# TiagoBsCastro/SLICER

Measured on AMD Instinct MI355X. Metric: particles/s deposited (TSC, 4096^2 map), higher is better.
Workload: dtype f32; 1 GPU; 512^3-particle GADGET-2 boxes (8 sub-files), 4 snapshots resident in HBM, 4096^2 TSC, 4 lens planes per pass, uniform; algo=auto, accum=f32, algo_mask=84, streams=1

## Files before the change

slicer_amd/csrc/binned_pass.cpp:

```cpp
#include "slicer_host.hpp"

#include <algorithm>
#include <cmath>
#include <cstring>

using namespace slicer;

namespace {

size_t acc_elem_size(int kind) { return (kind == kF64 || kind == kFixed64) ? 8 : 4; }

int zero_flush(slicer_handle h)
{
    ZeroList &Z = h->zero_list;
    if (Z.n == 1) {
        HIPCHK(h, hipMemsetAsync(Z.p[0], 0, Z.words[0] * 4, h->stream));
    } else if (Z.n > 1) {
        HIPCHK(h, launch_zero_many(Z, h->stream));
    }
    Z.n = 0;
    Z.quad0[0] = 0;
    return SLICER_OK;
}

// ... 83 lines not shown
                if (rc)
                    return rc;
                rc = zero_async(h, h->planes[p].acc[type].p, b);
                if (rc)
                    return rc;
            }
        }
        h->type_seen[type] = true;
    }
    return SLICER_OK;
}


int scatter_workgroups(slicer_handle h)
{
    return h->num_cus * std::max(1, h->opt.k3_per_cu);
}

int ensure_bin_workspace(slicer_handle h, bool has_mass, int group, int slot, uint64_t n, const BinGeom &G,
                         BinWorkspace &W)
{
    auto &Q = h->pg[group];
    const uint64_t nb = (n + G.batch - 1) / G.batch;
    const uint64_t region = (uint64_t)G.n_units * nb * G.region;
    const uint64_t nrec = n * (uint64_t)(G.region / G.batch);
    int rc;
    if ((rc = ensure(h, h->w_cxy, region * 8)) || (rc = ensure(h, h->w_cbin, region * 2)) ||
        (rc = ensure(h, h->w_hist, nb * (uint64_t)G.nbins * 4)) ||
        (rc = ensure(h, h->w_hist16, nb * (uint64_t)(G.nbins + 2) * 2)) ||
        (rc = ensure(h, h->w_total, (kMaxBins + kMaxBins / 32 + 1) * 4)) ||
        (rc = ensure(h, h->w_bcount, nb * kMaxUnits * 4)) || (rc = ensure(h, Q.w_sxy[slot], nrec * (has_mass ? 12 : 8))) ||
        (rc = ensure(h, Q.w_base[slot], (kMaxBins + 1) * 4)))
        return rc;
    if (has_mass && (rc = ensure(h, h->w_cm, region * 4)))
        return rc;
    W.cxy = (float2 *)h->w_cxy.p;
    W.cbin = (unsigned short *)h->w_cbin.p;
    W.cm = (float *)h->w_cm.p;
    W.sxy = (float2 *)Q.w_sxy[slot].p;
    W.sm = has_mass ? (float *)Q.w_sxy[slot].p : nullptr;
    W.hist = (unsigned *)h->w_hist.p;
    W.hist16 = (unsigned *)h->w_hist16.p;
    W.total = (unsigned *)h->w_total.p;
    W.base = (unsigned *)Q.w_base[slot].p;
    W.bcount = (unsigned *)h->w_bcount.p;
    return SLICER_OK;
}

bool sort2_geom(const BinGeom &G, int n_planes, BinGeom &G2, int &crow_log2)
{
    G2 = G;
    crow_log2 = 0;
    auto units = [&](int cl) { return n_planes * ((G.nty + (1 << cl) - 1) >> cl); };
    while (units(crow_log2) > 64 && (2 << crow_log2) * G.ntx <= kMaxCoarseTiles)
        crow_log2++;
    G2.rows_per_unit = 1 << crow_log2;
    G2.units_per_plane = (G.nty + G2.rows_per_unit - 1) / G2.rows_per_unit;
    G2.tiles_per_unit = G2.rows_per_unit * G.ntx;
    G2.n_units = n_planes * G2.units_per_plane;
    G2.nbins = G2.n_units * G2.tiles_per_unit;
    return G2.n_units <= kMaxCoarse && G2.tiles_per_unit <= kMaxCoarseTiles && G.region == G.batch && G.batch <= 32768;
// ... 326 lines not shown
```

slicer_amd/csrc/slicer_capi.cpp:

```cpp
#include "slicer_host.hpp"

#include <algorithm>
#include <cmath>
#include <cstdlib>
#include <cstring>
#include <new>

using namespace slicer;

namespace {

int env_int(const char *name, int dflt = 0)
{
    const char *v = getenv(name);
    return v && *v ? atoi(v) : dflt;
}

int copy_map_to_host(slicer_handle h, void *dst, const void *d_src, size_t bytes)
{
    HIPCHK(h, hipMemcpy(dst, d_src, bytes, hipMemcpyDeviceToHost));
    return SLICER_OK;
}

}
// ... 107 lines not shown
}

int slicer_destroy(slicer_handle h)
{
    if (!h)
        return SLICER_OK;
    (void)hipSetDevice(h->device);
    (void)hipStreamSynchronize(h->stream);
    prof_collect(h);
    thin_drop(h);
    pass_stream_return(h);
    for (auto e : h->ev_pool)
        (void)hipEventDestroy(e);
    for (auto &pl : h->planes) {
        release(pl.tot);
        release(pl.acc_shared);
        for (int t = 0; t < 6; t++) {
            release(pl.toti[t]);
            release(pl.acc[t]);
        }
    }
    if (h->d_sweep)
        (void)hipFree(h->d_sweep);
    for (DevBuf *b : {&h->w_cxy, &h->w_cbin, &h->w_cm, &h->w_hist, &h->w_hist16, &h->w_total, &h->w_bcount, &h->w_items,
                      &h->w_tcounts, &h->w_tbase, &h->w_urand, &h->w_randtab, &h->w_randstate, &h->w_randwaves, &h->w_c1, &h->w_sboff, &h->w_sbstart, &h->w_sbn})
        release(*b);
    for (auto &Q : h->pg) {
        release(Q.w_tot);
        for (int i = 0; i < kMaxPending; i++) {
            release(Q.w_sxy[i]);
            release(Q.w_base[i]);
            release(Q.w_ptab[i]);
        }
    }
    for (int i = 0; i < 2; i++) {
        if (h->h_stage[i]) (void)hipHostFree(h->h_stage[i]);
        if (h->d_stage[i]) (void)hipFree(h->d_stage[i]);
        if (h->h_mstage[i]) (void)hipHostFree(h->h_mstage[i]);
        if (h->d_mstage[i]) (void)hipFree(h->d_mstage[i]);
        if (h->stage_free[i]) (void)hipEventDestroy(h->stage_free[i]);
    }
    if (h->d_counts) (void)hipFree(h->d_counts);
    if (h->own) (void)hipStreamDestroy(h->own);
    delete h;
    return SLICER_OK;
}

// ... 484 lines not shown
```

slicer_amd/csrc/slicer_host.hpp:

```cpp
#pragma once
#include <hip/hip_runtime.h>

#include <cstdint>
#include <string>
#include <utility>
#include <vector>

#include "../../include/slicer_amd.h"
#include "slicer_kernels.hpp"

#pragma GCC visibility push(hidden)

struct DevBuf {
    void *p = nullptr;
    size_t cap = 0;
};

struct PlaneBufs {
    DevBuf tot;
    DevBuf toti[6];
    DevBuf acc[6];
    DevBuf acc_shared;
};

// ... 68 lines not shown
    unsigned long long *d_counts = nullptr;
    int *d_neg = nullptr;
    unsigned *d_maxmass = nullptr;
    bool type_seen[6] = {};
    bool shared_seen = false;
    int algo_mask = 0;
    bool neg_remote = false;
    int file_mode[6] = {};
    bool file_partial_flush[6] = {};
    unsigned file_serial = 0;
    float file_mconst[6] = {};
    int fixed_exp[6] = {};
    int fixed_exp_shared = 0;
    bool fixed_exp_set[6] = {};
    bool fixed_shared_set = false;

    float *h_stage[2] = {nullptr, nullptr};
    float *d_stage[2] = {nullptr, nullptr};
    float *h_mstage[2] = {nullptr, nullptr};
    float *d_mstage[2] = {nullptr, nullptr};
    hipEvent_t stage_free[2] = {nullptr, nullptr};
    uint64_t stage_cap = 0;

    DevBuf w_cxy, w_cbin, w_cm, w_hist, w_hist16, w_total, w_bcount, w_items;
    DevBuf w_c1, w_sboff, w_sbstart, w_sbn;
    std::vector<std::pair<double, bool>> box_verdicts;
    std::vector<std::pair<int, bool>> dl_verdicts;
    bool dl_quot_ok = false;
    unsigned *d_sweep = nullptr;
    DevBuf w_tcounts, w_tbase, w_urand;
    std::vector<float> h_urand;
    DevBuf w_randtab, w_randstate, w_randwaves;
    bool rand_tab_ready = false;
    bool rand_on_device = false;
    slicer::ZeroList zero_list{};
    bool zero_collect = false;
    bool rand_private = false;
    uint32_t rand_state[31] = {};
    bool rand_pass = false;
    struct ThinChunk {
        int file, type;
        DevBuf pos, mass;
        uint64_t n;
    };
    struct ThinFile {
        slicer_file_desc file;
        int mode[6];
// ... 96 lines not shown
```

slicer_amd/csrc/slicer_kernels.hpp:

```cpp
#pragma once
#include <hip/hip_runtime.h>
#include <stdint.h>

#include "slicer_device.hpp"

namespace slicer {

enum Mas { kTSC = 0, kNGP = 1 };
enum Acc { kF32 = 0, kF64 = 1, kFixed64 = 2, kCountU32 = 3,
           kF32I = 4, kF64I = 5 };

struct Targets {
    void *acc[kMaxPlanes];
    unsigned long long *nsel[kMaxPlanes];
    int *neg_flag;
    unsigned *max_mass;
};

struct LaunchCfg {
    int mas;
    int acc;
    bool has_mass;
};

hipError_t launch_direct(const LaunchCfg &cfg, const float *d_pos, const float *d_mass, uint64_t n,
                         const PassParams &P, const Targets &T, hipStream_t s);
// ... 53 lines not shown
                                int *neg_flag, hipStream_t s);

struct BinGeom {
    int tw_log2, th_log2;
    int ntx, nty;
    int tiles_per_unit;
    int units_per_plane;
    int rows_per_unit;
    int n_units;
    int nbins;
    int batch;
    int region;
};
constexpr int kMaxUnits = 32;
constexpr int kMaxBins = 32768;

struct BinWorkspace {
    float2 *c1;
    unsigned *sb_off, *sb_n;
    unsigned short *sb_start;
    unsigned *ptab;
    unsigned *item_tot;
    unsigned *tot;
    float2 *cxy;
    unsigned short *cbin;
    float *cm;
    float2 *sxy;
    float *sm;
    unsigned *hist16;
    unsigned *hist;
    unsigned *total;
    unsigned *base;
    unsigned *bcount;
};

struct K1Args {
    const float *pos;
    const float *mass;
    uint64_t n;
    float2 *cxy;
    unsigned short *cbin;
    float *cm;
    unsigned *hist16;
    unsigned *bcount;
    int *neg_flag;
    unsigned long long *nsel;
    float rb, boxf;
    float ws[3], wo[3];
    float c0f[3];
    float rcase;
    int face;
    float zlo[4], zlast;
    int n_planes, vec, ngp;
    int stack;
    float k_ra, eps_ra, k_dec, eps_dec;
    double series_max, lim, inv_fov;
    double nn_d;
    float nn_f;
    int nn;
    int pow2;
    int tw_log2, th_log2, ntx, tiles_per_unit, units_per_plane, rows_per_unit, n_units, nbins, batch;
    int ntx_log2, tpu_log2;
    int sort2, crow_log2;
    float2 *c1;
    unsigned *sb_off;
// ... 61 lines not shown
```

slicer_amd/csrc/slicer_project_bin.hip:

```cpp
#include "slicer_binned_common.hpp"

#pragma clang fp contract(off)

namespace slicer {

namespace {

#ifndef SLICER_K1_BLOCK
#define SLICER_K1_BLOCK 512
#endif
#ifndef SLICER_K1_WAVES_PER_SIMD
#define SLICER_K1_WAVES_PER_SIMD 4
#endif
constexpr int kK1Block = SLICER_K1_BLOCK;
#ifndef SLICER_K1_PER_THREAD
#define SLICER_K1_PER_THREAD 4
#endif
constexpr int kPerThread = SLICER_K1_PER_THREAD;
static_assert(kPerThread == 4 || kPerThread == 2, "load_round handles 2 or 4 particles per lane");
constexpr int kRound = kK1Block * kPerThread;
constexpr int kWaves = kK1Block / 64;
constexpr int kWaveQ = 64 * kPerThread + 64;

struct RawRound {
// ... 159 lines not shown
        A.sb_off[sg] = blockIdx.x * (unsigned)A.batch + off;
    lds_barrier();
    if (tid < nu)
        St.cnt[tid] = 0;
    if (tid == 3 * 64)
        *St.n = 0;
    float2 *out = A.c1 + (size_t)blockIdx.x * (size_t)A.batch + off;
    for (unsigned j = tid; j < n; j += kK1Block)
        out[j] = St.rec[St.perm[j]];
    off += n;
    slot++;
    lds_barrier();
}

enum { kEmitGeneric = 0,
       kEmitLean = 1,
       kEmitSort2 = 2,
       kEmitLeanNgp = 3,
       kEmitLeanMass = 4 };

template <int MODE, bool POW2>
__device__ __forceinline__ void emit_record(const K1Args &A, unsigned *s_hist, unsigned *s_out, unsigned *s_cnt, bool valid,
                                            int plane, float xs, float ys, int gx, int gy, unsigned idx_in_batch,
                                            uint64_t b0, float2 *out_wg, unsigned unit_stride)
{
    constexpr bool LEAN = MODE == kEmitLean || MODE == kEmitLeanNgp || MODE == kEmitLeanMass;
    const bool ngp = MODE == kEmitLeanNgp || (!LEAN && A.ngp != 0);
    const int nn = A.nn;
    bool emit = valid;
    if (ngp) {
        emit = valid && gx >= 0 && gx < nn && gy >= 0 && gy < nn;
        if (valid && !emit)
            atomicAdd(&s_cnt[plane], 1u);
    }
    gx = min(max(gx, 0), nn - 1);
    gy = min(max(gy, 0), nn - 1);
    if (MODE == kEmitSort2 || (MODE == kEmitGeneric && A.sort2)) {
        const Stage St = stage_of(s_hist);
        const unsigned coarse = (unsigned)plane * (unsigned)A.units_per_plane + ((unsigned)(gy >> A.th_log2) >> A.crow_log2);
        const unsigned long long em = __ballot(emit);
        if (em != 0ull) {
            const int lead = (int)__builtin_ctzll(em);
            unsigned base = 0;
            if ((int)lane_id() == lead)
                base = atomicAdd(St.n, (unsigned)__popcll(em));
            base = (unsigned)__builtin_amdgcn_readlane((int)base, lead);
            if (emit) {
                const unsigned idx = base + (unsigned)__popcll(em & ((1ull << lane_id()) - 1ull));
                const unsigned r = atomicAdd(&St.cnt[coarse], 1u);
                St.rec[idx] = make_float2(xs, ys);
                St.bin[idx] = (unsigned char)coarse;
                St.rank[idx] = (unsigned short)r;
            }
        }
        return;
    }
    if (emit) {
        const unsigned ty = (unsigned)(gy >> A.th_log2), tx = (unsigned)(gx >> A.tw_log2);
        unsigned band = 0, trow = ty;
        if (!LEAN && A.units_per_plane > 1) {
            band = ty / (unsigned)A.rows_per_unit;
            trow = ty - band * (unsigned)A.rows_per_unit;
        }
        const unsigned unit = LEAN ? (unsigned)plane : (unsigned)plane * (unsigned)A.units_per_plane + band;
        const bool shifts = LEAN && POW2;
        const unsigned tile_in_unit = shifts ? (trow << A.ntx_log2) | tx : trow * (unsigned)A.ntx + tx;
        const unsigned bin = shifts ? (unit << A.tpu_log2) | tile_in_unit : unit * (unsigned)A.tiles_per_unit + tile_in_unit;
        const unsigned o = atomicAdd(&s_out[unit], 1u);
        const unsigned idx = unit * unit_stride + o;
        out_wg[idx] = make_float2(xs, ys);
        A.cbin[(size_t)blockIdx.x * (size_t)A.batch + idx] = (unsigned short)tile_in_unit;
        if (MODE == kEmitLeanMass || (!LEAN && A.mass != nullptr))
            A.cm[(size_t)blockIdx.x * (size_t)A.batch + idx] = A.mass[b0 + idx_in_batch];
        atomicAdd(&s_hist[bin >> 1], 1u << ((bin & 1u) * 16u));
    }
}

__device__ SLICER_SLOWPATH bool process_exact(const K1Kernarg *Kk, unsigned *s_hist, unsigned *s_out, unsigned *s_cnt,
                                              unsigned idx_in_batch, uint64_t b0, float2 *out_wg, unsigned unit_stride)
{
    const PassParams P = Kk->P;
    const K1Args A = Kk->A;
    const float *r = A.pos + 3 * (b0 + idx_in_batch);
    float x, y, z;
    transform(r[0], r[1], r[2], P, x, y, z);
    const bool neg = (x < 0.0f) | (y < 0.0f) | (z < 0.0f);
    for (int p = 0; p < P.n_planes; p++) {
        if (!(z >= P.zlo[p] && z < P.zhi[p]))
            continue;
        float xs, ys;
        if (project<0>(x, y, z, 0, 0, P, xs, ys)) {
            const int gx = P.pow2 ? grid_index<true>(xs, P) : grid_index<false>(xs, P);
            const int gy = P.pow2 ? grid_index<true>(ys, P) : grid_index<false>(ys, P);
            emit_record<kEmitGeneric, false>(A, s_hist, s_out, s_cnt, true, p, xs, ys, gx, gy, idx_in_batch, b0, out_wg, unit_stride);
        }
    }
    return neg;
}

template <bool POW2, int MODE>
__device__ __forceinline__ void decide_emit(const K1Args &A, unsigned *s_hist, unsigned *s_out, unsigned *s_cnt,
                                            unsigned *s_exc, unsigned *s_nexc, bool have, float ez, double sn, double tn,
                                            double dec, double ra, unsigned tag, uint64_t b0, float2 *out_wg,
                                            unsigned unit_stride)
{
    float xs = 0.f, ys = 0.f;
    const double adec = fabs(dec), ara = fabs(ra);
    const double sx = fma(dec, A.inv_fov, 0.5), sy = fma(ra, A.inv_fov, 0.5);
    const bool dx = round_decided(sx, kMapWindow, xs), dy = round_decided(sy, kMapWindow, ys);
    bool undecided = !(fabs(sn) <= A.series_max && fabs(tn) <= A.series_max && ez > 0.0f) ||
                     fabs(adec - A.lim) <= kAngWindow || fabs(ara - A.lim) <= kAngWindow || !dx || !dy;
    int gx, gy;
    if (POW2) {
        gx = (int)floorf(xs * A.nn_f);
        gy = (int)floorf(ys * A.nn_f);
    } else {
        const double tx = (double)xs * A.nn_d, ty = (double)ys * A.nn_d;
        const double fx = floor(tx), fy = floor(ty);
        undecided = undecided || tx == fx || ty == fy;
        gx = (int)fx;
        gy = (int)fy;
    }
    if (have && undecided)
        s_exc[min(atomicAdd(s_nexc, 1u), kExcCap - 1)] = tag >> 3;
    const bool valid = have && !undecided && adec <= A.lim && ara <= A.lim;
    emit_record<MODE, POW2>(A, s_hist, s_out, s_cnt, valid, (int)(tag & 7u), xs, ys, gx, gy, tag >> 3, b0, out_wg, unit_stride);
}

template <int SERIES, bool POW2, int MODE>
__device__ __forceinline__ void project_emit(const K1Args &A, unsigned *s_hist, unsigned *s_out, unsigned *s_cnt,
                                             unsigned *s_exc, unsigned *s_nexc, bool have, float ex, float ey, float ez,
                                             unsigned tag, uint64_t b0, float2 *out_wg, unsigned unit_stride)
{
    const double X = (double)ex - 0.5, Y = (double)ey - 0.5, Z = (double)ez;
    const double R2 = fma(Y, Y, Z * Z);
    const double sn = X * rsqrt_fast(R2);
    const double tn = Y * rcp_fast(Z);
    double dec, ra;
    atan_small_pair<SERIES>(sn, tn, dec, ra);
    decide_emit<POW2, MODE>(A, s_hist, s_out, s_cnt, s_exc, s_nexc, have, ez, sn, tn, dec, ra, tag, b0, out_wg, unit_stride);
}

template <int SERIES, bool POW2, int MODE>
__device__ __forceinline__ void project_emit2(const K1Args &A, unsigned *s_hist, unsigned *s_out, unsigned *s_cnt,
                                              unsigned *s_exc, unsigned *s_nexc, const bool *have, const float *ex,
                                              const float *ey, const float *ez, const unsigned *tag, uint64_t b0, float2 *out_wg, unsigned unit_stride)
{
    double t[4], ang[4];
#pragma unroll
    for (int j = 0; j < 2; j++) {
        const double X = (double)ex[j] - 0.5, Y = (double)ey[j] - 0.5, Z = (double)ez[j];
        const double R2 = fma(Y, Y, Z * Z);
        t[2 * j] = X * rsqrt_fast(R2);
        t[2 * j + 1] = Y * rcp_fast(Z);
    }
    atan_small_quad<SERIES>(t, ang);
#pragma unroll
    for (int j = 0; j < 2; j++)
        decide_emit<POW2, MODE>(A, s_hist, s_out, s_cnt, s_exc, s_nexc, have[j], ez[j], t[2 * j], t[2 * j + 1], ang[2 * j],
                          ang[2 * j + 1], tag[j], b0, out_wg, unit_stride);
}

template <int FACE, int SERIES, bool STACK, bool POW2, int MODE>
__global__ __launch_bounds__(kK1Block, SLICER_K1_WAVES_PER_SIMD) void k_project_bin_fast(K1Kernarg K)
{
    constexpr bool SORT2 = MODE == kEmitSort2;
    static_assert(!(STACK && SORT2), "the two-level sort runs without the wave stacks");
    const K1Args &A = K.A;
    extern __shared__ __attribute__((aligned(16))) unsigned smem[];
// ... 11 lines not shown
        s_hist[i] = 0;
    if (tid < kMaxPlanes)
        s_cnt[tid] = 0;
    if (tid < kMaxUnits)
        s_out[tid] = 0;
    if (tid == 0) {
        s_neg = 0;
        s_nexc = 0;
    }
    if (SORT2) {
        const Stage St = stage_of(smem);
        if (tid < kMaxCoarse) {
            St.cnt[tid] = 0;
            St.tot[tid] = 0;
        }
        if (tid == 0)
            *St.n = 0;
    }
    __syncthreads();
    unsigned st_off = 0, st_slot = 0;

    const uint64_t b0 = (uint64_t)blockIdx.x * A.batch;
    const uint64_t b1 = dmin<uint64_t>(A.n, b0 + A.batch);
    float2 *const out_wg = A.cxy + (size_t)blockIdx.x * (size_t)A.batch;
    const unsigned unit_stride = gridDim.x * (unsigned)A.batch;
    unsigned top = 0;

    const uint64_t w0 = b0 + (uint64_t)wave * (64 * kPerThread);
    RawRound cur;
    const __amdgpu_buffer_rsrc_t rsrc = batch_rsrc(A.pos, b0, b1);
    uint64_t i0 = w0 + (uint64_t)kPerThread * lane;
    int nvalid = i0 < b1 ? (int)dmin<uint64_t>(kPerThread, b1 - i0) : 0;
    load_round(rsrc, (unsigned)(i0 - b0), cur);

    const uint64_t lim = SORT2 ? b1 + (w0 - b0) : b1;
    for (uint64_t r0 = w0; r0 < lim; r0 += kRound) {
        const uint64_t i1 = i0 + kRound;
        const bool more = r0 + kRound < lim;
        const int nvalid1 = (more && i1 < b1) ? (int)dmin<uint64_t>(kPerThread, b1 - i1) : 0;

        static_assert(kPerThread % 2 == 0, "particles are projected in pairs");
        float px[kPerThread], py[kPerThread], pz[kPerThread];
        bool psel[kPerThread];
        unsigned ptag[kPerThread];
        {
#pragma unroll
            for (int k = 0; k < kPerThread; k++) {
// ... 117 lines not shown
                atomicAdd(&A.item_tot[(size_t)(blockIdx.x / kSort2Blocks) * A.n_units + tid], c);
                atomicAdd(&s_cnt[tid / A.units_per_plane], c);
            }
        }
        __syncthreads();
        if (tid < A.n_planes && s_cnt[tid])
            atomicAdd(A.nsel + 6 * tid, (unsigned long long)s_cnt[tid]);
        return;
    }
    unsigned *row = A.hist16 + (size_t)blockIdx.x * hist_words;
    for (int i = tid; i < hist_words; i += kK1Block)
        row[i] = s_hist[i];
    if (tid < A.n_units)
        A.bcount[(size_t)tid * gridDim.x + blockIdx.x] = s_out[tid];
    if (tid == 0 && s_neg)
        atomicOr(A.neg_flag, 1);
    if (A.ngp && tid < A.n_planes && s_cnt[tid])
        atomicAdd(A.nsel + 6 * tid, (unsigned long long)s_cnt[tid]);
}

template <int MAS, bool POW2, bool HAS_MASS, int SERIES, bool REP>
__global__ __launch_bounds__(kK1Block, SLICER_K1_WAVES_PER_SIMD) void k_project_bin_general(
    const float *__restrict__ pos, const float *__restrict__ mass, uint64_t n, int vec, PassParams P, BinGeom G,
    float2 *__restrict__ cxy, unsigned short *__restrict__ cbin, float *__restrict__ cm, unsigned *__restrict__ hist16,
    unsigned *__restrict__ bcount, Targets T)
{
    extern __shared__ unsigned smem[];
    unsigned *s_hist = smem;
    const int hist_words = (G.nbins + 1) >> 1;
    const int tid = threadIdx.x;
    const unsigned lane = lane_id();
    const int wave = tid >> 6;
    float4 *q4 = reinterpret_cast<float4 *>(smem + ((hist_words + 3) & ~3)) + (size_t)wave * kWaveQ;
    __shared__ unsigned s_out[kMaxUnits], s_cnt[kMaxPlanes];
    __shared__ int s_neg;

    for (int i = tid; i < hist_words; i += kK1Block)
        s_hist[i] = 0;
    if (tid < kMaxPlanes)
        s_cnt[tid] = 0;
    if (tid < kMaxUnits)
        s_out[tid] = 0;
    if (tid == 0)
        s_neg = 0;
    __syncthreads();

    const uint64_t b0 = (uint64_t)blockIdx.x * G.batch;
// ... 29 lines not shown
                    valid = true;
                    int gx = grid_index<POW2>(xs, P);
                    int gy = grid_index<POW2>(ys, P);
                    const int nn = P.nn;
                    if (MAS == kNGP) {
                        emit = gx >= 0 && gx < nn && gy >= 0 && gy < nn;
                    } else {
                        emit = true;
                        gx = gx < 0 ? 0 : (gx >= nn ? nn - 1 : gx);
                        gy = gy < 0 ? 0 : (gy >= nn ? nn - 1 : gy);
                    }
                    cell_to_tile(gx, gy, plane, G, unit, tile_in_unit);
                    bin = unit * (unsigned)G.tiles_per_unit + tile_in_unit;
                    if (HAS_MASS)
                        m = mass[b0 + (tag >> 10)];
                }
            }
            top -= take;
            if (MAS == kNGP && valid && !emit)
                atomicAdd(&s_cnt[plane], 1u);
            if (emit) {
                const unsigned o = atomicAdd(&s_out[unit], 1u);
                const uint64_t dst = ((uint64_t)unit * gridDim.x + blockIdx.x) * (uint64_t)G.region + o;
                cxy[dst] = make_float2(xs, ys);
                cbin[dst] = (unsigned short)tile_in_unit;
                if (HAS_MASS)
                    cm[dst] = m;
                atomicAdd(&s_hist[bin >> 1], 1u << ((bin & 1u) * 16u));
            }
        }
    };

    for (uint64_t r0 = w0; r0 < b1; r0 += kRound) {
        const uint64_t i1 = i0 + kRound;
        const bool more = r0 + kRound < b1;
        const int nvalid1 = (more && i1 < b1) ? (int)dmin<uint64_t>(kPerThread, b1 - i1) : 0;
        load_round(rsrc, (unsigned)(i1 - b0), nxt);

        if (!REP) {
#pragma unroll
            for (int k = 0; k < kPerThread; k++) {
                float x, y, z;
                transform(cur.v[3 * k], cur.v[3 * k + 1], cur.v[3 * k + 2], P, x, y, z);
                const bool live = k < nvalid;
                neg |= live & ((x < 0.0f) | (y < 0.0f) | (z < 0.0f));
                int pl = -1;
                if (P.n_planes <= 4) {
#pragma unroll
                    for (int p = 0; p < 4; p++)
                        if (z >= P.zlo[p] && z < P.zhi[p])
// ... 158 lines not shown
            if (s9) K1F(9, false, kEmitLeanMass); else K1F(15, false, kEmitLeanMass);
        } else if (lean) {
            if (s9) K1F(9, false, kEmitLean); else K1F(15, false, kEmitLean);
        } else {
            if (s9) K1F(9, false, kEmitGeneric); else K1F(15, false, kEmitGeneric);
        }
    }
#undef K1F_
#undef K1F
    return hipGetLastError();
}

template <int MAS, bool POW2, bool HAS_MASS, int SERIES>
static hipError_t launch_k1_general(bool vec, const float *pos, const float *mass, uint64_t n, const PassParams &P,
                                    const BinGeom &G, const BinWorkspace &W, const Targets &T, hipStream_t s)
{
    const int nb = (int)((n + G.batch - 1) / G.batch);
    const size_t lds = project_bin_lds_bytes(G, HAS_MASS);
    hipError_t e;
    if (G.region != G.batch) {
        auto kern = k_project_bin_general<MAS, POW2, HAS_MASS, SERIES, true>;
        if ((e = set_lds(kern, lds)) != hipSuccess)
            return e;
        kern<<<nb, kK1Block, lds, s>>>(pos, mass, n, vec ? 1 : 0, P, G, W.cxy, W.cbin, W.cm, W.hist16, W.bcount, T);
    } else {
        auto kern = k_project_bin_general<MAS, POW2, HAS_MASS, SERIES, false>;
        if ((e = set_lds(kern, lds)) != hipSuccess)
            return e;
        kern<<<nb, kK1Block, lds, s>>>(pos, mass, n, vec ? 1 : 0, P, G, W.cxy, W.cbin, W.cm, W.hist16, W.bcount, T);
    }
    return hipGetLastError();
}

hipError_t launch_project_bin(const LaunchCfg &cfg, bool fast, const float *d_pos, const float *d_mass, uint64_t n,
                              const PassParams &P, const K1Args &A0, const BinGeom &G, const BinWorkspace &W,
                              const Targets &T, hipStream_t s)
{
    const bool vec = (reinterpret_cast<uintptr_t>(d_pos) & 15u) == 0 && (G.batch % 4) == 0;
    const bool pow2 = P.pow2 != 0;
    bool s9 = P.series_max < 0.2;
    if (fast) {
        s9 = A0.series_max < 0.2;
        K1Args A = A0;
        A.pos = d_pos;
        A.mass = cfg.has_mass ? d_mass : nullptr;
        A.n = n;
        A.vec = vec ? 1 : 0;
        A.ngp = cfg.mas == kNGP;
        A.cxy = W.cxy;
        A.cbin = W.cbin;
        A.cm = W.cm;
        A.hist16 = W.hist16;
        A.bcount = W.bcount;
        A.neg_flag = T.neg_flag;
        A.nsel = T.nsel[0];
        A.tw_log2 = G.tw_log2, A.th_log2 = G.th_log2, A.ntx = G.ntx, A.tiles_per_unit = G.tiles_per_unit;
        auto log2_exact = [](int v) {
            int l = 0;
            while ((1 << l) < v)
                l++;
            return (1 << l) == v ? l : -1;
        };
        A.ntx_log2 = log2_exact(G.ntx), A.tpu_log2 = log2_exact(G.tiles_per_unit);
        A.units_per_plane = G.units_per_plane, A.rows_per_unit = G.rows_per_unit, A.n_units = G.n_units;
        A.nbins = G.nbins, A.batch = G.batch;
        A.c1 = W.c1;
        A.sb_off = W.sb_off;
        A.sb_start = W.sb_start;
        A.sb_n = W.sb_n;
        A.item_tot = W.item_tot;
        if (A.sort2)
            A.stack = 0;
        const int nb = (int)((n + G.batch - 1) / G.batch);
        const size_t lds = A.sort2 ? project_bin_sort2_lds_bytes() : project_bin_lds_bytes(G, cfg.has_mass);
// ... 25 lines not shown
```

slicer_amd/csrc/slicer_sort.hip:

```cpp
#include "slicer_binned_common.hpp"

#pragma clang fp contract(off)

namespace slicer {


constexpr int kScanBins = 32;
constexpr int kScanSegs = 1024 / kScanBins;

__global__ __launch_bounds__(1024) void k_scan_blocks(const unsigned short *__restrict__ hist16,
                                                      unsigned *__restrict__ prefix, unsigned *__restrict__ lex,
                                                      unsigned *__restrict__ gsum, int nblocks, int nbins)
{
    __shared__ unsigned s_seg[kScanSegs][kScanBins];
    const int bl = threadIdx.x % kScanBins, seg = threadIdx.x / kScanBins;
    const int bin = blockIdx.x * kScanBins + bl;
    const size_t stride16 = (size_t)((nbins + 1) >> 1) * 2;
    const int per = (nblocks + kScanSegs - 1) / kScanSegs;
    const int lo = seg * per, hi = lo + per < nblocks ? lo + per : nblocks;
    constexpr int kKeep = 16;
    unsigned short keep[kKeep];
    const bool kept = per <= kKeep;
    unsigned sum = 0;
    if (bin < nbins) {
// ... 37 lines not shown
            const unsigned y = (unsigned)__shfl_up((int)x, d, kScanBins);
            if (bl >= d)
                x += y;
        }
        if (bin < nbins)
            lex[bin] = x - tot;
        if (bl == kScanBins - 1)
            gsum[blockIdx.x] = x;
    }
}

#ifndef SLICER_K3_BLOCK
#define SLICER_K3_BLOCK 512
#endif
constexpr int kSortBlock = SLICER_K3_BLOCK;
constexpr int kSortBatch = 8192;
#ifndef SLICER_K3_STAGE
#define SLICER_K3_STAGE 4096
#endif
#ifndef SLICER_K3_WAVES
#define SLICER_K3_WAVES 4
#endif
constexpr int kSortStage = SLICER_K3_STAGE;

__device__ __forceinline__ unsigned block_exclusive_scan(unsigned v, unsigned *s_wave )
{
    unsigned x = v;
#pragma unroll
    for (int d = 1; d < 64; d <<= 1) {
        const unsigned y = (unsigned)__shfl_up((int)x, d);
        if ((int)lane_id() >= d)
            x += y;
    }
    const int w = threadIdx.x >> 6;
    if (lane_id() == 63)
        s_wave[w] = x;
    lds_barrier();
    unsigned off = 0;
    for (int k = 0; k < w; k++)
        off += s_wave[k];
    lds_barrier();
    return off + x - v;
}

template <bool HAS_MASS>
__global__ __launch_bounds__(kSortBlock, SLICER_K3_WAVES) void k_bin_scatter(const float2 *__restrict__ cxy,
                                                            const unsigned short *__restrict__ cbin,
                                                            const float *__restrict__ cm,
                                                            const unsigned *__restrict__ hist16w,
                                                            const unsigned *__restrict__ prefix,
                                                            const unsigned *__restrict__ lex,
                                                            const unsigned *__restrict__ gsum,
                                                            unsigned *__restrict__ base,
                                                            const unsigned *__restrict__ bcount, int nblocks,
                                                            BinGeom G, float2 *__restrict__ sxy,
                                                            float *__restrict__ sm, int count_planes, Targets T)
{
    extern __shared__ unsigned smem_sc[];
    const int tpp = G.tiles_per_unit;
    const int tw = (tpp + 1) >> 1;
    unsigned *cnt = smem_sc;
    unsigned *pos = cnt + tw;
    unsigned *cur = pos + tpp;
    float2 *sorted_xy = reinterpret_cast<float2 *>(cur + tpp + (tw & 1));
    unsigned short *sorted_tile = reinterpret_cast<unsigned short *>(sorted_xy + kSortStage);
    float *sorted_m = reinterpret_cast<float *>(sorted_tile + kSortStage);
    __shared__ unsigned s_wave[kSortBlock / 64];
    __shared__ unsigned s_gp[kMaxBins / kScanBins + 1];

    const int tid = threadIdx.x;
    {
// ... 14 lines not shown
                s_gp[g] = e;
            e += v[j];
        }
        if (tid == kSortBlock - 1)
            s_gp[ngroups] = e;
        lds_barrier();
        if (blockIdx.x == 0) {
            for (int i = tid; i <= G.nbins; i += kSortBlock)
                base[i] = i < G.nbins ? s_gp[i / kScanBins] + lex[i] : s_gp[ngroups];
            if (tid < count_planes) {
                const int bpp = G.units_per_plane * G.tiles_per_unit;
                auto at = [&](int i) { return i < G.nbins ? s_gp[i / kScanBins] + lex[i] : s_gp[ngroups]; };
                const unsigned c = at((tid + 1) * bpp) - at(tid * bpp);
                if (c)
                    atomicAdd(T.nsel[tid], (unsigned long long)c);
            }
        }
    }
    const int per_unit = 8 * ((nblocks + 7) / 8);
    const int per_xcd = per_unit / 8;
    const int per = (tpp + kSortBlock - 1) / kSortBlock;
    auto get16 = [](const unsigned *tab, unsigned t) { return (tab[t >> 1] >> ((t & 1u) * 16u)) & 0xFFFFu; };
    constexpr int R = kSortBatch / kSortBlock;
    float mass_max = 0.0f;
    for (int item = blockIdx.x; item < G.n_units * per_unit; item += gridDim.x) {
        const int plane = item / per_unit;
        const int u = item % per_unit;
        const int lb = (u & 7) * per_xcd + (u >> 3);
        if (lb >= nblocks)
            continue;
        const unsigned count = bcount[(size_t)plane * nblocks + lb];
        if (count == 0)
            continue;
        lds_barrier();
        const unsigned *row = prefix + (size_t)lb * G.nbins + (size_t)plane * tpp;
        const unsigned *lrow = lex + (size_t)plane * tpp;
        const unsigned bin0 = (unsigned)plane * (unsigned)tpp;
        for (int i = tid; i < tpp; i += kSortBlock)
            cur[i] = s_gp[(bin0 + (unsigned)i) / kScanBins] + lrow[i] + row[i];
        const uint64_t r0 = ((uint64_t)plane * nblocks + lb) * (uint64_t)G.region;

        const bool single = count <= (unsigned)kSortBatch && (((unsigned)plane * (unsigned)tpp) & 1u) == 0u;
        for (unsigned s0 = 0; s0 < count; s0 += kSortBatch) {
            const unsigned nsub = count - s0 < (unsigned)kSortBatch ? count - s0 : (unsigned)kSortBatch;
            if (!single) {
                for (int i = tid; i < tw; i += kSortBlock)
                    cnt[i] = 0;
                lds_barrier();
            }
            unsigned tile[R];
            float2 xy[R];
            float m[R];
#pragma unroll
            for (int k = 0; k < R; k++) {
                const unsigned i = (unsigned)k * kSortBlock + tid;
                if (i < nsub) {
                    tile[k] = cbin[r0 + s0 + i];
                    xy[k] = cxy[r0 + s0 + i];
                    if (HAS_MASS)
                        m[k] = cm[r0 + s0 + i];
                    if (!single)
                        atomicAdd(&cnt[tile[k] >> 1], 1u << ((tile[k] & 1u) * 16u));
                }
            }
            if (single) {
                const unsigned *hrow =
                    hist16w + (size_t)lb * (size_t)((G.nbins + 1) >> 1) + (((size_t)plane * tpp) >> 1);
                for (int i = tid; i < tw; i += kSortBlock)
                    cnt[i] = (i == tw - 1 && (tpp & 1)) ? (hrow[i] & 0xFFFFu) : hrow[i];
            }
            lds_barrier();
            {
                unsigned sum = 0;
                for (int j = 0; j < per; j++) {
                    const unsigned t = (unsigned)(tid * per + j);
                    if ((int)t < tpp)
                        sum += get16(cnt, t);
                }
                unsigned e = block_exclusive_scan(sum, s_wave);
                for (int j = 0; j < per; j++) {
                    const unsigned t = (unsigned)(tid * per + j);
                    if ((int)t < tpp) {
                        pos[t] = e;
                        cur[t] -= e;
                        e += get16(cnt, t);
                    }
                }
            }
            lds_barrier();
#pragma unroll
            for (int k = 0; k < R; k++) {
                const unsigned i = (unsigned)k * kSortBlock + tid;
                if (i < nsub)
                    tile[k] |= atomicAdd(&pos[tile[k]], 1u) << 16;
                else
                    tile[k] = 0xFFFF0000u;
            }
            if (HAS_MASS) {
#pragma unroll
                for (int k = 0; k < R; k++)
                    if ((unsigned)k * kSortBlock + tid < nsub)
                        mass_max = fmaxf(mass_max, cap_mass(m[k]));
            }
            for (unsigned lo = 0; lo < nsub; lo += kSortStage) {
                lds_barrier();
#pragma unroll
                for (int k = 0; k < R; k++) {
                    const unsigned q = (tile[k] >> 16) - lo;
                    if (q < (unsigned)kSortStage) {
                        sorted_xy[q] = xy[k];
                        sorted_tile[q] = (unsigned short)(tile[k] & 0xFFFFu);
                        if (HAS_MASS)
                            sorted_m[q] = m[k];
                    }
                }
                lds_barrier();
                const unsigned hi = nsub - lo < (unsigned)kSortStage ? nsub - lo : (unsigned)kSortStage;
                for (unsigned q = tid; q < hi; q += kSortBlock) {
                    const unsigned dst = cur[sorted_tile[q]] + lo + q;
                    if (HAS_MASS) {
                        const float2 v = sorted_xy[q];
                        reinterpret_cast<Rec3 *>(sxy)[dst] = Rec3{v.x, v.y, sorted_m[q]};
                    } else {
                        sxy[dst] = sorted_xy[q];
// ... 210 lines not shown
{
    (void)cfg, (void)n_planes, (void)T;
    const int ngroups = (G.nbins + kScanBins - 1) / kScanBins;
    k_scan_blocks<<<ngroups, 1024, 0, s>>>(reinterpret_cast<const unsigned short *>(W.hist16), W.hist, W.total,
                                           W.total + kMaxBins, nblocks, G.nbins);
    return hipGetLastError();
}

size_t scatter_lds_bytes(const BinGeom &G, bool has_mass)
{
    const size_t tpp = (size_t)G.tiles_per_unit, tw = (tpp + 1) >> 1;
    return 4 * (tw + 2 * tpp + (tw & 1)) + (size_t)kSortStage * (8 + 2 + (has_mass ? 4 : 0));
}

hipError_t launch_bin_scatter(const LaunchCfg &cfg, int nblocks, int n_planes, int max_workgroups, const BinGeom &G,
                              const BinWorkspace &W, const Targets &T, hipStream_t s)
{
    const bool has_mass = cfg.has_mass;
    const size_t lds = scatter_lds_bytes(G, has_mass);
    const int items = G.n_units * 8 * ((nblocks + 7) / 8);
    const int nwg = std::min(items, std::max(8, max_workgroups / 8 * 8));
    const int count_planes = n_planes;
    return launch_with_lds(has_mass ? k_bin_scatter<true> : k_bin_scatter<false>, nwg, kSortBlock, lds, 0, s,
                           W.cxy, W.cbin, W.cm, W.hist16, W.hist, W.total, W.total + kMaxBins, W.base, W.bcount, nblocks, G,
                           W.sxy, W.sm, count_planes, T);
}

size_t sort2_lds_bytes(int slots_per_group, int tiles_per_unit)
{
    return (size_t)kS2Cap * 9 + 4 * ((size_t)slots_per_group * 2 + 1 + 4 * (size_t)tiles_per_unit) + 2 * (kS2Cap / 64);
}

hipError_t launch_sort2(int nblocks, int slots_per_group, int ngroups, int max_workgroups, const PassParams &P,
                        const BinGeom &G, const BinWorkspace &W, hipStream_t s)
{
    const size_t lds = sort2_lds_bytes(slots_per_group, G.tiles_per_unit);
    const int nitems = G.n_units * ngroups;
    const int nwg = std::min(nitems, std::max(std::max(8, max_workgroups), (nitems + kS2MaxMine - 1) / kS2MaxMine));
    return launch_with_lds(P.pow2 ? k_sort2<true> : k_sort2<false>, nwg, kS2Block, lds, 0, s, W.c1, W.sb_off,
                           W.sb_start, W.sb_n, nblocks, slots_per_group, ngroups, G, P, W.sxy, W.ptab, W.item_tot, W.tot);
}

}
```

Baseline: 55.79 billion particles/s.

## Pack projection-to-scatter hand-off into interleaved 12/16-byte records

```diff
diff --git a/slicer_amd/csrc/binned_pass.cpp b/slicer_amd/csrc/binned_pass.cpp
--- a/slicer_amd/csrc/binned_pass.cpp
+++ b/slicer_amd/csrc/binned_pass.cpp
@@ -129,21 +129,17 @@
 {
     auto &Q = h->pg[group];
     const uint64_t nb = (n + G.batch - 1) / G.batch;
-    const uint64_t region = (uint64_t)G.n_units * nb * G.region;
+    const uint64_t crec_bytes = handoff_bytes(G.n_units, n, G.batch, G.region, has_mass);
     const uint64_t nrec = n * (uint64_t)(G.region / G.batch);
     int rc;
-    if ((rc = ensure(h, h->w_cxy, region * 8)) || (rc = ensure(h, h->w_cbin, region * 2)) ||
+    if ((rc = ensure(h, h->w_crec, crec_bytes)) ||
         (rc = ensure(h, h->w_hist, nb * (uint64_t)G.nbins * 4)) ||
         (rc = ensure(h, h->w_hist16, nb * (uint64_t)(G.nbins + 2) * 2)) ||
         (rc = ensure(h, h->w_total, (kMaxBins + kMaxBins / 32 + 1) * 4)) ||
         (rc = ensure(h, h->w_bcount, nb * kMaxUnits * 4)) || (rc = ensure(h, Q.w_sxy[slot], nrec * (has_mass ? 12 : 8))) ||
         (rc = ensure(h, Q.w_base[slot], (kMaxBins + 1) * 4)))
         return rc;
-    if (has_mass && (rc = ensure(h, h->w_cm, region * 4)))
-        return rc;
-    W.cxy = (float2 *)h->w_cxy.p;
-    W.cbin = (unsigned short *)h->w_cbin.p;
-    W.cm = (float *)h->w_cm.p;
+    W.crec = h->w_crec.p;
     W.sxy = (float2 *)Q.w_sxy[slot].p;
     W.sm = has_mass ? (float *)Q.w_sxy[slot].p : nullptr;
     W.hist = (unsigned *)h->w_hist.p;
diff --git a/slicer_amd/csrc/handoff_layout.hpp b/slicer_amd/csrc/handoff_layout.hpp
--- /dev/null
+++ b/slicer_amd/csrc/handoff_layout.hpp
@@ -0,0 +1,32 @@
+#pragma once
+#include <stdint.h>
+
+namespace slicer {
+
+struct __attribute__((packed, aligned(4))) HandRec3 {
+    float x, y;
+    uint32_t tile;
+};
+struct __attribute__((aligned(16))) HandRec4 {
+    float x, y;
+    uint32_t tile;
+    float m;
+};
+static_assert(sizeof(HandRec3) == 12 && sizeof(HandRec4) == 16, "hand-off records are 12 / 16 bytes");
+
+constexpr uint64_t handoff_record_bytes(bool has_mass) { return has_mass ? sizeof(HandRec4) : sizeof(HandRec3); }
+
+constexpr uint64_t handoff_records(int n_units, uint64_t n, int batch, int region)
+{
+    return (uint64_t)n_units * ((n + (uint64_t)batch - 1) / (uint64_t)batch) * (uint64_t)region;
+}
+constexpr uint64_t handoff_bytes(int n_units, uint64_t n, int batch, int region, bool has_mass)
+{
+    return handoff_records(n_units, n, batch, region) * handoff_record_bytes(has_mass);
+}
+constexpr uint64_t handoff_region_offset(int unit, uint64_t nblocks, uint64_t lb, int region, bool has_mass)
+{
+    return ((uint64_t)unit * nblocks + lb) * (uint64_t)region * handoff_record_bytes(has_mass);
+}
+
+}
diff --git a/slicer_amd/csrc/slicer_capi.cpp b/slicer_amd/csrc/slicer_capi.cpp
--- a/slicer_amd/csrc/slicer_capi.cpp
+++ b/slicer_amd/csrc/slicer_capi.cpp
@@ -153,7 +153,7 @@
     }
     if (h->d_sweep)
         (void)hipFree(h->d_sweep);
-    for (DevBuf *b : {&h->w_cxy, &h->w_cbin, &h->w_cm, &h->w_hist, &h->w_hist16, &h->w_total, &h->w_bcount, &h->w_items,
+    for (DevBuf *b : {&h->w_crec, &h->w_hist, &h->w_hist16, &h->w_total, &h->w_bcount, &h->w_items,
                       &h->w_tcounts, &h->w_tbase, &h->w_urand, &h->w_randtab, &h->w_randstate, &h->w_randwaves, &h->w_c1, &h->w_sboff, &h->w_sbstart, &h->w_sbn})
         release(*b);
     for (auto &Q : h->pg) {
diff --git a/slicer_amd/csrc/slicer_host.hpp b/slicer_amd/csrc/slicer_host.hpp
--- a/slicer_amd/csrc/slicer_host.hpp
+++ b/slicer_amd/csrc/slicer_host.hpp
@@ -114,7 +114,7 @@
     hipEvent_t stage_free[2] = {nullptr, nullptr};
     uint64_t stage_cap = 0;
 
-    DevBuf w_cxy, w_cbin, w_cm, w_hist, w_hist16, w_total, w_bcount, w_items;
+    DevBuf w_crec, w_hist, w_hist16, w_total, w_bcount, w_items;
     DevBuf w_c1, w_sboff, w_sbstart, w_sbn;
     std::vector<std::pair<double, bool>> box_verdicts;
     std::vector<std::pair<int, bool>> dl_verdicts;
diff --git a/slicer_amd/csrc/slicer_kernels.hpp b/slicer_amd/csrc/slicer_kernels.hpp
--- a/slicer_amd/csrc/slicer_kernels.hpp
+++ b/slicer_amd/csrc/slicer_kernels.hpp
@@ -2,6 +2,7 @@
 #include <hip/hip_runtime.h>
 #include <stdint.h>
 
+#include "handoff_layout.hpp"
 #include "slicer_device.hpp"
 
 namespace slicer {
@@ -101,9 +102,7 @@
     unsigned *ptab;
     unsigned *item_tot;
     unsigned *tot;
-    float2 *cxy;
-    unsigned short *cbin;
-    float *cm;
+    void *crec;
     float2 *sxy;
     float *sm;
     unsigned *hist16;
@@ -117,9 +116,7 @@
     const float *pos;
     const float *mass;
     uint64_t n;
-    float2 *cxy;
-    unsigned short *cbin;
-    float *cm;
+    void *crec;
     unsigned *hist16;
     unsigned *bcount;
     int *neg_flag;
diff --git a/slicer_amd/csrc/slicer_project_bin.hip b/slicer_amd/csrc/slicer_project_bin.hip
--- a/slicer_amd/csrc/slicer_project_bin.hip
+++ b/slicer_amd/csrc/slicer_project_bin.hip
@@ -205,7 +205,7 @@
 template <int MODE, bool POW2>
 __device__ __forceinline__ void emit_record(const K1Args &A, unsigned *s_hist, unsigned *s_out, unsigned *s_cnt, bool valid,
                                             int plane, float xs, float ys, int gx, int gy, unsigned idx_in_batch,
-                                            uint64_t b0, float2 *out_wg, unsigned unit_stride)
+                                            uint64_t b0, void *out_wg, unsigned unit_stride)
 {
     constexpr bool LEAN = MODE == kEmitLean || MODE == kEmitLeanNgp || MODE == kEmitLeanMass;
     const bool ngp = MODE == kEmitLeanNgp || (!LEAN && A.ngp != 0);
@@ -251,16 +251,16 @@
         const unsigned bin = shifts ? (unit << A.tpu_log2) | tile_in_unit : unit * (unsigned)A.tiles_per_unit + tile_in_unit;
         const unsigned o = atomicAdd(&s_out[unit], 1u);
         const unsigned idx = unit * unit_stride + o;
-        out_wg[idx] = make_float2(xs, ys);
-        A.cbin[(size_t)blockIdx.x * (size_t)A.batch + idx] = (unsigned short)tile_in_unit;
         if (MODE == kEmitLeanMass || (!LEAN && A.mass != nullptr))
-            A.cm[(size_t)blockIdx.x * (size_t)A.batch + idx] = A.mass[b0 + idx_in_batch];
+            reinterpret_cast<HandRec4 *>(out_wg)[idx] = HandRec4{xs, ys, tile_in_unit, A.mass[b0 + idx_in_batch]};
+        else
+            reinterpret_cast<HandRec3 *>(out_wg)[idx] = HandRec3{xs, ys, tile_in_unit};
         atomicAdd(&s_hist[bin >> 1], 1u << ((bin & 1u) * 16u));
     }
 }
 
 __device__ SLICER_SLOWPATH bool process_exact(const K1Kernarg *Kk, unsigned *s_hist, unsigned *s_out, unsigned *s_cnt,
-                                              unsigned idx_in_batch, uint64_t b0, float2 *out_wg, unsigned unit_stride)
+                                              unsigned idx_in_batch, uint64_t b0, void *out_wg, unsigned unit_stride)
 {
     const PassParams P = Kk->P;
     const K1Args A = Kk->A;
@@ -284,7 +284,7 @@
 template <bool POW2, int MODE>
 __device__ __forceinline__ void decide_emit(const K1Args &A, unsigned *s_hist, unsigned *s_out, unsigned *s_cnt,
                                             unsigned *s_exc, unsigned *s_nexc, bool have, float ez, double sn, double tn,
-                                            double dec, double ra, unsigned tag, uint64_t b0, float2 *out_wg,
+                                            double dec, double ra, unsigned tag, uint64_t b0, void *out_wg,
                                             unsigned unit_stride)
 {
     float xs = 0.f, ys = 0.f;
@@ -313,7 +313,7 @@
 template <int SERIES, bool POW2, int MODE>
 __device__ __forceinline__ void project_emit(const K1Args &A, unsigned *s_hist, unsigned *s_out, unsigned *s_cnt,
                                              unsigned *s_exc, unsigned *s_nexc, bool have, float ex, float ey, float ez,
-                                             unsigned tag, uint64_t b0, float2 *out_wg, unsigned unit_stride)
+                                             unsigned tag, uint64_t b0, void *out_wg, unsigned unit_stride)
 {
     const double X = (double)ex - 0.5, Y = (double)ey - 0.5, Z = (double)ez;
     const double R2 = fma(Y, Y, Z * Z);
@@ -327,7 +327,7 @@
 template <int SERIES, bool POW2, int MODE>
 __device__ __forceinline__ void project_emit2(const K1Args &A, unsigned *s_hist, unsigned *s_out, unsigned *s_cnt,
                                               unsigned *s_exc, unsigned *s_nexc, const bool *have, const float *ex,
-                                              const float *ey, const float *ez, const unsigned *tag, uint64_t b0, float2 *out_wg, unsigned unit_stride)
+                                              const float *ey, const float *ez, const unsigned *tag, uint64_t b0, void *out_wg, unsigned unit_stride)
 {
     double t[4], ang[4];
 #pragma unroll
@@ -385,7 +385,8 @@
 
     const uint64_t b0 = (uint64_t)blockIdx.x * A.batch;
     const uint64_t b1 = dmin<uint64_t>(A.n, b0 + A.batch);
-    float2 *const out_wg = A.cxy + (size_t)blockIdx.x * (size_t)A.batch;
+    const bool rec4 = MODE == kEmitLeanMass || ((MODE == kEmitGeneric || MODE == kEmitSort2) && A.mass != nullptr);
+    void *const out_wg = static_cast<char *>(A.crec) + (size_t)blockIdx.x * (size_t)A.batch * handoff_record_bytes(rec4);
     const unsigned unit_stride = gridDim.x * (unsigned)A.batch;
     unsigned top = 0;
 
@@ -549,7 +550,7 @@
 template <int MAS, bool POW2, bool HAS_MASS, int SERIES, bool REP>
 __global__ __launch_bounds__(kK1Block, SLICER_K1_WAVES_PER_SIMD) void k_project_bin_general(
     const float *__restrict__ pos, const float *__restrict__ mass, uint64_t n, int vec, PassParams P, BinGeom G,
-    float2 *__restrict__ cxy, unsigned short *__restrict__ cbin, float *__restrict__ cm, unsigned *__restrict__ hist16,
+    void *__restrict__ crec, unsigned *__restrict__ hist16,
     unsigned *__restrict__ bcount, Targets T)
 {
     extern __shared__ unsigned smem[];
@@ -625,10 +626,10 @@
             if (emit) {
                 const unsigned o = atomicAdd(&s_out[unit], 1u);
                 const uint64_t dst = ((uint64_t)unit * gridDim.x + blockIdx.x) * (uint64_t)G.region + o;
-                cxy[dst] = make_float2(xs, ys);
-                cbin[dst] = (unsigned short)tile_in_unit;
                 if (HAS_MASS)
-                    cm[dst] = m;
+                    reinterpret_cast<HandRec4 *>(crec)[dst] = HandRec4{xs, ys, tile_in_unit, m};
+                else
+                    reinterpret_cast<HandRec3 *>(crec)[dst] = HandRec3{xs, ys, tile_in_unit};
                 atomicAdd(&s_hist[bin >> 1], 1u << ((bin & 1u) * 16u));
             }
         }
@@ -833,12 +834,12 @@
         auto kern = k_project_bin_general<MAS, POW2, HAS_MASS, SERIES, true>;
         if ((e = set_lds(kern, lds)) != hipSuccess)
             return e;
-        kern<<<nb, kK1Block, lds, s>>>(pos, mass, n, vec ? 1 : 0, P, G, W.cxy, W.cbin, W.cm, W.hist16, W.bcount, T);
+        kern<<<nb, kK1Block, lds, s>>>(pos, mass, n, vec ? 1 : 0, P, G, W.crec, W.hist16, W.bcount, T);
     } else {
         auto kern = k_project_bin_general<MAS, POW2, HAS_MASS, SERIES, false>;
         if ((e = set_lds(kern, lds)) != hipSuccess)
             return e;
-        kern<<<nb, kK1Block, lds, s>>>(pos, mass, n, vec ? 1 : 0, P, G, W.cxy, W.cbin, W.cm, W.hist16, W.bcount, T);
+        kern<<<nb, kK1Block, lds, s>>>(pos, mass, n, vec ? 1 : 0, P, G, W.crec, W.hist16, W.bcount, T);
     }
     return hipGetLastError();
 }
@@ -858,9 +859,7 @@
         A.n = n;
         A.vec = vec ? 1 : 0;
         A.ngp = cfg.mas == kNGP;
-        A.cxy = W.cxy;
-        A.cbin = W.cbin;
-        A.cm = W.cm;
+        A.crec = W.crec;
         A.hist16 = W.hist16;
         A.bcount = W.bcount;
         A.neg_flag = T.neg_flag;
diff --git a/slicer_amd/csrc/slicer_sort.hip b/slicer_amd/csrc/slicer_sort.hip
--- a/slicer_amd/csrc/slicer_sort.hip
+++ b/slicer_amd/csrc/slicer_sort.hip
@@ -83,6 +83,10 @@
 #define SLICER_K3_WAVES 4
 #endif
 constexpr int kSortStage = SLICER_K3_STAGE;
+#ifndef SLICER_K3_CONSEC
+#define SLICER_K3_CONSEC 0
+#endif
+constexpr bool kSortConsec = SLICER_K3_CONSEC != 0;
 
 __device__ __forceinline__ unsigned block_exclusive_scan(unsigned v, unsigned *s_wave )
 {
@@ -105,9 +109,7 @@
 }
 
 template <bool HAS_MASS>
-__global__ __launch_bounds__(kSortBlock, SLICER_K3_WAVES) void k_bin_scatter(const float2 *__restrict__ cxy,
-                                                            const unsigned short *__restrict__ cbin,
-                                                            const float *__restrict__ cm,
+__global__ __launch_bounds__(kSortBlock, SLICER_K3_WAVES) void k_bin_scatter(const void *__restrict__ crec,
                                                             const unsigned *__restrict__ hist16w,
                                                             const unsigned *__restrict__ prefix,
                                                             const unsigned *__restrict__ lex,
@@ -168,6 +170,12 @@
     const int per = (tpp + kSortBlock - 1) / kSortBlock;
     auto get16 = [](const unsigned *tab, unsigned t) { return (tab[t >> 1] >> ((t & 1u) * 16u)) & 0xFFFFu; };
     constexpr int R = kSortBatch / kSortBlock;
+    constexpr bool CONSEC = kSortConsec && !HAS_MASS;
+    static_assert(R % 4 == 0, "a lane takes its records four at a time");
+    auto rec_index = [&](int k) {
+        return CONSEC ? 4u * ((unsigned)(k >> 2) * kSortBlock + (unsigned)tid) + (unsigned)(k & 3)
+                      : (unsigned)k * kSortBlock + (unsigned)tid;
+    };
     float mass_max = 0.0f;
     for (int item = blockIdx.x; item < G.n_units * per_unit; item += gridDim.x) {
         const int plane = item / per_unit;
@@ -197,17 +205,43 @@
             unsigned tile[R];
             float2 xy[R];
             float m[R];
-#pragma unroll
-            for (int k = 0; k < R; k++) {
-                const unsigned i = (unsigned)k * kSortBlock + tid;
-                if (i < nsub) {
-                    tile[k] = cbin[r0 + s0 + i];
-                    xy[k] = cxy[r0 + s0 + i];
-                    if (HAS_MASS)
-                        m[k] = cm[r0 + s0 + i];
-                    if (!single)
+            if (HAS_MASS) {
+                const HandRec4 *src = static_cast<const HandRec4 *>(crec) + (r0 + s0);
+#pragma unroll
+                for (int k = 0; k < R; k++) {
+                    const unsigned i = rec_index(k);
+                    const HandRec4 v = src[i < nsub ? i : nsub - 1u];
+                    xy[k] = make_float2(v.x, v.y);
+                    tile[k] = v.tile;
+                    m[k] = v.m;
+                }
+            } else if (CONSEC) {
+                const uint4 *src = reinterpret_cast<const uint4 *>(static_cast<const HandRec3 *>(crec) + (r0 + s0));
+#pragma unroll
+                for (int g = 0; g < R / 4; g++) {
+                    unsigned q = (unsigned)g * kSortBlock + tid;
+                    q = 4u * q < nsub ? q : (nsub - 1u) >> 2;
+                    const uint4 a = src[3u * q], b = src[3u * q + 1u], c = src[3u * q + 2u];
+                    xy[4 * g] = make_float2(__uint_as_float(a.x), __uint_as_float(a.y)), tile[4 * g] = a.z;
+                    xy[4 * g + 1] = make_float2(__uint_as_float(a.w), __uint_as_float(b.x)), tile[4 * g + 1] = b.y;
+                    xy[4 * g + 2] = make_float2(__uint_as_float(b.z), __uint_as_float(b.w)), tile[4 * g + 2] = c.x;
+                    xy[4 * g + 3] = make_float2(__uint_as_float(c.y), __uint_as_float(c.z)), tile[4 * g + 3] = c.w;
+                }
+            } else {
+                const HandRec3 *src = static_cast<const HandRec3 *>(crec) + (r0 + s0);
+#pragma unroll
+                for (int k = 0; k < R; k++) {
+                    const unsigned i = rec_index(k);
+                    const HandRec3 v = src[i < nsub ? i : nsub - 1u];
+                    xy[k] = make_float2(v.x, v.y);
+                    tile[k] = v.tile;
+                }
+            }
+            if (!single) {
+#pragma unroll
+                for (int k = 0; k < R; k++)
+                    if (rec_index(k) < nsub)
                         atomicAdd(&cnt[tile[k] >> 1], 1u << ((tile[k] & 1u) * 16u));
-                }
             }
             if (single) {
                 const unsigned *hrow =
@@ -236,7 +270,7 @@
             lds_barrier();
 #pragma unroll
             for (int k = 0; k < R; k++) {
-                const unsigned i = (unsigned)k * kSortBlock + tid;
+                const unsigned i = rec_index(k);
                 if (i < nsub)
                     tile[k] |= atomicAdd(&pos[tile[k]], 1u) << 16;
                 else
@@ -245,7 +279,7 @@
             if (HAS_MASS) {
 #pragma unroll
                 for (int k = 0; k < R; k++)
-                    if ((unsigned)k * kSortBlock + tid < nsub)
+                    if (rec_index(k) < nsub)
                         mass_max = fmaxf(mass_max, cap_mass(m[k]));
             }
             for (unsigned lo = 0; lo < nsub; lo += kSortStage) {
@@ -502,7 +536,7 @@
     const int nwg = std::min(items, std::max(8, max_workgroups / 8 * 8));
     const int count_planes = n_planes;
     return launch_with_lds(has_mass ? k_bin_scatter<true> : k_bin_scatter<false>, nwg, kSortBlock, lds, 0, s,
-                           W.cxy, W.cbin, W.cm, W.hist16, W.hist, W.total, W.total + kMaxBins, W.base, W.bcount, nblocks, G,
+                           W.crec, W.hist16, W.hist, W.total, W.total + kMaxBins, W.base, W.bcount, nblocks, G,
                            W.sxy, W.sm, count_planes, T);
 }
 
```

Result: no change. 55.25 billion particles/s (-1.0%).
